# vnoz/Mutual-Information-MultiModal

Hardware: AMD Instinct MI355X
Metric: img-txt pairs/sec (MI critic fwd+bwd), global-batch InfoNCE (higher is better)
Workload: dtype bf16; 1 GPU; BASELINE configs[3]: global-batch infonce (reference semantics), bilinear critic fwd+bwd, B_global=4096, d=512; global_batch=4096, embed_dim=512, critic=bilinear, estimator=infonce, parallelism=single GPU, boundary=fp32 embeddings in, fp32 gradients out, hip_graph=False, graph_mode=none (direct C-ABI calls)

## Files before the change

mutual-information-multimodal_amd/csrc/mi_bilinear_flash.h:

```cpp
#pragma once
#include <type_traits>

#include "mi_common.h"

namespace mi {

#ifdef MI_STAMPS
#define MI_FL_STAMP(slot)                                                                       \
  do {                                                                                          \
    __builtin_amdgcn_sched_barrier(0);                                                          \
    if (threadIdx.x == 0 && g_stamps) g_stamps[(size_t)blockIdx.x * 16 + (slot)] = __builtin_amdgcn_s_memtime(); \
    __builtin_amdgcn_sched_barrier(0);                                                          \
  } while (0)
#else
#define MI_FL_STAMP(slot) do {} while (0)
#endif

#ifndef MI_FL_DIAG
#define MI_FL_DIAG 0
#endif
constexpr int kFlDiag = MI_FL_DIAG;
constexpr int kFlRows = 128;
constexpr int kFlBN = 32;
constexpr int kFlStages = 4;
constexpr float kFlThr = 60.0f;
constexpr int kFlMaxTilesPerSplit = 64;

struct FlashProblem {
  const bf16_t* q;
  const bf16_t* kv;
  const int64_t* sid_q;
  const int64_t* sid_kv;
  int64_t m, n;
  int64_t diag;
  int n_rb;
  int n_split;
  int tiles_per_split;
  const unsigned char* dup;
  float* slab;
  Partial* rec;
};
struct FlashArgs {
  FlashProblem p[2];
  int n_problems;
  int n_combo;
  int xcd_rows;
  int diag;
  int slab_f16;
  int no_index_mask;
};

template <int D>
struct FlashCfg {
  static constexpr int NK = D / 16;
  static constexpr int NT = D / 32;
  static constexpr int RB = D * 2;
  static constexpr int CPR = RB / 16;
  static constexpr int RPP = 1024 / RB;
  static constexpr int STAGE = kFlBN * RB;
  static constexpr int PIECES = STAGE / 1024 / 4;
  static constexpr int SID_OFF = kFlStages * STAGE;
  static constexpr size_t SMEM = (size_t)SID_OFF + (size_t)kFlMaxTilesPerSplit * kFlBN * 8;
  static constexpr int QA = NT >= 16 ? NK / 2 : 0;
  static constexpr int OA = NT >= 16 ? 12 : NT;
  static_assert(D == 128 || D == 256 || D == 512, "unsupported embedding width");
};

__host__ __device__ constexpr int fl_swz(int row) { return ((row & 3) << 2) | ((row >> 2) & 3); }

__device__ __forceinline__ float wave_max_uniform(float v) {
  int x;
#define MI_DPP_MAX(ctrl, rmask)                                                        \
  x = __builtin_amdgcn_update_dpp(__float_as_int(v), __float_as_int(v), ctrl, rmask, 0xF, false); \
  v = fmaxf(v, __int_as_float(x));
  MI_DPP_MAX(0xB1, 0xF)
  MI_DPP_MAX(0x4E, 0xF)
  MI_DPP_MAX(0x141, 0xF)
  MI_DPP_MAX(0x140, 0xF)
  MI_DPP_MAX(0x142, 0xA)
  MI_DPP_MAX(0x143, 0xC)
#undef MI_DPP_MAX
  return __int_as_float(__builtin_amdgcn_readlane(__float_as_int(v), 63));
}

__device__ __forceinline__ void fl_dma16(unsigned voff, const void* sbase, unsigned lds_addr) {
  unsigned keep;
  const uintptr_t b = (uintptr_t)sbase;
  const unsigned blo = __builtin_amdgcn_readfirstlane((unsigned)b), bhi = __builtin_amdgcn_readfirstlane((unsigned)(b >> 32));
  sbase = (const void*)(((uintptr_t)bhi << 32) | blo);
  lds_addr = __builtin_amdgcn_readfirstlane(lds_addr);
  asm volatile("s_mov_b32 %0, m0\n\ts_mov_b32 m0, %3\n\ts_nop 1\n\tglobal_load_lds_dwordx4 %1, %2\n\ts_mov_b32 m0, %0"
               : "=&s"(keep)
               : "v"(voff), "s"(sbase), "s"(lds_addr)
               : "memory");
}

template <int LOFF>
__device__ __forceinline__ void fl_dma_set_m0(unsigned lds_base) {
  asm volatile("s_add_u32 m0, %0, %1" : : "s"(lds_base), "n"(LOFF) : "scc");
}
template <int GOFF, int XORC>
__device__ __forceinline__ void fl_dma16_at(unsigned vlane_w, const void* sbase) {
  unsigned voff;
  asm volatile("v_xor_b32 %0, %3, %1\n\tglobal_load_lds_dwordx4 %0, %2 offset:%4"
               : "=&v"(voff)
               : "v"(vlane_w), "s"(sbase), "n"(XORC), "n"(GOFF)
               : "memory");
}

__device__ __forceinline__ float fl_max3(float a, float b, float c) {
  float d;
  asm("v_max3_f32 %0, %1, %2, %3" : "=v"(d) : "v"(a), "v"(b), "v"(c));
  return d;
}

__device__ __forceinline__ void fl_v_exp(const float& x) { asm volatile("v_exp_f32 %0, %0" : : "v"(x)); }
__device__ __forceinline__ void fl_v_add(const float& acc, const float& p) { asm volatile("v_add_f32 %0, %0, %1" : : "v"(acc), "v"(p)); }
__device__ __forceinline__ void fl_v_opaque(float& x) { asm volatile("; fl_opaque" : "+v"(x)); }
__device__ __forceinline__ unsigned fl_v_cvt_pk(const float& lo, const float& hi) {
  unsigned d;
  asm volatile("v_cvt_pk_bf16_f32 %0, %1, %2" : "=v"(d) : "v"(lo), "v"(hi));
  return d;
}
__device__ __forceinline__ void fl_v_prescale(float& x, const float& s, const float& off) {
  asm volatile("v_fmamk_f32 %0, %1, 0x3fb8aa3b, %2" : "=v"(x) : "v"(s), "v"(off));
}
__device__ __forceinline__ void fl_v_max(float& d, const float& a, const float& b) {
  asm volatile("v_max_f32 %0, %1, %2" : "=v"(d) : "v"(a), "v"(b));
}
__device__ __forceinline__ void fl_v_max3(float& d, const float& a, const float& b) {
  asm volatile("v_max3_f32 %0, %0, %1, %2" : "+v"(d) : "v"(a), "v"(b));
}
template <int STEP, bool NOP>
__device__ __forceinline__ void fl_dpp_max(const float& v) {
#define MI_FL_DPP(ctrl)                                                                            \
  if constexpr (NOP) asm volatile("s_nop 1\n\tv_max_f32_dpp %0, %0, %0 " ctrl : : "v"(v));          \
  else asm volatile("v_max_f32_dpp %0, %0, %0 " ctrl : : "v"(v))
  if constexpr (STEP == 0) { MI_FL_DPP("quad_perm:[1,0,3,2] row_mask:0xf bank_mask:0xf"); }
  else if constexpr (STEP == 1) { MI_FL_DPP("quad_perm:[2,3,0,1] row_mask:0xf bank_mask:0xf"); }
  else if constexpr (STEP == 2) { MI_FL_DPP("row_half_mirror row_mask:0xf bank_mask:0xf"); }
  else if constexpr (STEP == 3) { MI_FL_DPP("row_mirror row_mask:0xf bank_mask:0xf"); }
  else if constexpr (STEP == 4) { MI_FL_DPP("row_bcast:15 row_mask:0xa bank_mask:0xf"); }
  else { MI_FL_DPP("row_bcast:31 row_mask:0xc bank_mask:0xf"); }
#undef MI_FL_DPP
}

template <int N>
__device__ __forceinline__ void fl_wait_vmcnt_barrier() {
  asm volatile("s_waitcnt vmcnt(%0)\n\ts_barrier" ::"n"(N) : "memory");
}

template <int B, int E, class F>
__device__ __forceinline__ void fl_static_for(F&& f) {
  if constexpr (B < E) {
    f(std::integral_constant<int, B>{});
    fl_static_for<B + 1, E>(f);
  }
}

constexpr int kFlRing = 9;
constexpr int kFlAhead = 8;

template <int SLOT, int OFF>
__device__ __forceinline__ void fl_ring_read_s(bf16x8& f, int addr) {
  static_assert(OFF >= 0 && OFF < 65536, "ds offset field");
  if constexpr (SLOT == 0)
    asm volatile("ds_read_b128 v[216:219], %1 offset:%c2" : "={v[216:219]}"(f) : "v"(addr), "i"(OFF));
  else if constexpr (SLOT == 1)
    asm volatile("ds_read_b128 v[220:223], %1 offset:%c2" : "={v[220:223]}"(f) : "v"(addr), "i"(OFF));
  else if constexpr (SLOT == 2)
    asm volatile("ds_read_b128 v[224:227], %1 offset:%c2" : "={v[224:227]}"(f) : "v"(addr), "i"(OFF));
  else if constexpr (SLOT == 3)
    asm volatile("ds_read_b128 v[228:231], %1 offset:%c2" : "={v[228:231]}"(f) : "v"(addr), "i"(OFF));
  else if constexpr (SLOT == 4)
    asm volatile("ds_read_b128 v[232:235], %1 offset:%c2" : "={v[232:235]}"(f) : "v"(addr), "i"(OFF));
  else if constexpr (SLOT == 5)
    asm volatile("ds_read_b128 v[236:239], %1 offset:%c2" : "={v[236:239]}"(f) : "v"(addr), "i"(OFF));
  else if constexpr (SLOT == 6)
    asm volatile("ds_read_b128 v[240:243], %1 offset:%c2" : "={v[240:243]}"(f) : "v"(addr), "i"(OFF));
  else if constexpr (SLOT == 7)
    asm volatile("ds_read_b128 v[244:247], %1 offset:%c2" : "={v[244:247]}"(f) : "v"(addr), "i"(OFF));
  else if constexpr (SLOT == 8)
    asm volatile("ds_read_b128 v[248:251], %1 offset:%c2" : "={v[248:251]}"(f) : "v"(addr), "i"(OFF));
  else if constexpr (SLOT == 9)
    asm volatile("ds_read_b128 v[252:255], %1 offset:%c2" : "={v[252:255]}"(f) : "v"(addr), "i"(OFF));
}
template <int SLOT, int OFF_LO, int OFF_HI>
__device__ __forceinline__ void fl_ring_read_v(bf16x8& f, int addr_lo, int addr_hi) {
  static_assert(OFF_LO >= 0 && OFF_HI < 65536, "ds offset field");
  if constexpr (SLOT == 0)
    asm volatile("ds_read_b64_tr_b16 v[216:217], %1 offset:%c3\n\tds_read_b64_tr_b16 v[218:219], %2 offset:%c4"
                 : "={v[216:219]}"(f) : "v"(addr_lo), "v"(addr_hi), "i"(OFF_LO), "i"(OFF_HI));
  else if constexpr (SLOT == 1)
    asm volatile("ds_read_b64_tr_b16 v[220:221], %1 offset:%c3\n\tds_read_b64_tr_b16 v[222:223], %2 offset:%c4"
                 : "={v[220:223]}"(f) : "v"(addr_lo), "v"(addr_hi), "i"(OFF_LO), "i"(OFF_HI));
  else if constexpr (SLOT == 2)
    asm volatile("ds_read_b64_tr_b16 v[224:225], %1 offset:%c3\n\tds_read_b64_tr_b16 v[226:227], %2 offset:%c4"
                 : "={v[224:227]}"(f) : "v"(addr_lo), "v"(addr_hi), "i"(OFF_LO), "i"(OFF_HI));
  else if constexpr (SLOT == 3)
    asm volatile("ds_read_b64_tr_b16 v[228:229], %1 offset:%c3\n\tds_read_b64_tr_b16 v[230:231], %2 offset:%c4"
                 : "={v[228:231]}"(f) : "v"(addr_lo), "v"(addr_hi), "i"(OFF_LO), "i"(OFF_HI));
  else if constexpr (SLOT == 4)
    asm volatile("ds_read_b64_tr_b16 v[232:233], %1 offset:%c3\n\tds_read_b64_tr_b16 v[234:235], %2 offset:%c4"
                 : "={v[232:235]}"(f) : "v"(addr_lo), "v"(addr_hi), "i"(OFF_LO), "i"(OFF_HI));
  else if constexpr (SLOT == 5)
    asm volatile("ds_read_b64_tr_b16 v[236:237], %1 offset:%c3\n\tds_read_b64_tr_b16 v[238:239], %2 offset:%c4"
                 : "={v[236:239]}"(f) : "v"(addr_lo), "v"(addr_hi), "i"(OFF_LO), "i"(OFF_HI));
  else if constexpr (SLOT == 6)
    asm volatile("ds_read_b64_tr_b16 v[240:241], %1 offset:%c3\n\tds_read_b64_tr_b16 v[242:243], %2 offset:%c4"
                 : "={v[240:243]}"(f) : "v"(addr_lo), "v"(addr_hi), "i"(OFF_LO), "i"(OFF_HI));
  else if constexpr (SLOT == 7)
    asm volatile("ds_read_b64_tr_b16 v[244:245], %1 offset:%c3\n\tds_read_b64_tr_b16 v[246:247], %2 offset:%c4"
                 : "={v[244:247]}"(f) : "v"(addr_lo), "v"(addr_hi), "i"(OFF_LO), "i"(OFF_HI));
  else if constexpr (SLOT == 8)
    asm volatile("ds_read_b64_tr_b16 v[248:249], %1 offset:%c3\n\tds_read_b64_tr_b16 v[250:251], %2 offset:%c4"
                 : "={v[248:251]}"(f) : "v"(addr_lo), "v"(addr_hi), "i"(OFF_LO), "i"(OFF_HI));
  else if constexpr (SLOT == 9)
    asm volatile("ds_read_b64_tr_b16 v[252:253], %1 offset:%c3\n\tds_read_b64_tr_b16 v[254:255], %2 offset:%c4"
                 : "={v[252:255]}"(f) : "v"(addr_lo), "v"(addr_hi), "i"(OFF_LO), "i"(OFF_HI));
}
template <int WAIT>
__device__ __forceinline__ void fl_wait_lgkm() {
  if constexpr (kFlDiag & 16) return;
  if constexpr (WAIT >= 0) asm volatile("s_waitcnt lgkmcnt(%c0)" ::"i"(WAIT) : "memory");
}
template <bool B_IN_ACC, bool FIRST, int WAIT>
__device__ __forceinline__ void fl_mfma_s(f32x16& acc, const bf16x8& a, const bf16x8& b) {
  fl_wait_lgkm<WAIT>();
  if constexpr (FIRST) {
    if constexpr (B_IN_ACC)
      asm volatile("v_mfma_f32_32x32x16_bf16 %0, %1, %2, 0" : "=v"(acc) : "v"(a), "a"(b));
    else
      asm volatile("v_mfma_f32_32x32x16_bf16 %0, %1, %2, 0" : "=v"(acc) : "v"(a), "v"(b));
  } else {
    if constexpr (B_IN_ACC)
      asm volatile("v_mfma_f32_32x32x16_bf16 %0, %1, %2, %0" : : "v"(acc), "v"(a), "a"(b));
    else
      asm volatile("v_mfma_f32_32x32x16_bf16 %0, %1, %2, %0" : : "v"(acc), "v"(a), "v"(b));
  }
}
template <bool ACC_IN_ACC, bool NOP, int WAIT, class AT>
__device__ __forceinline__ void fl_mfma_o(f32x16& acc, const AT& a, const bf16x8& b) {
  static_assert(sizeof(AT) == 16, "a 32x32x16 bf16 operand is four registers");
  fl_wait_lgkm<WAIT>();
  if constexpr (NOP) {
    if constexpr (ACC_IN_ACC)
      asm volatile("s_nop 1\n\tv_mfma_f32_32x32x16_bf16 %0, %1, %2, %0" : "+a"(acc) : "v"(a), "v"(b));
    else
      asm volatile("s_nop 1\n\tv_mfma_f32_32x32x16_bf16 %0, %1, %2, %0" : "+v"(acc) : "v"(a), "v"(b));
  } else {
    if constexpr (ACC_IN_ACC)
      asm volatile("v_mfma_f32_32x32x16_bf16 %0, %1, %2, %0" : "+a"(acc) : "v"(a), "v"(b));
    else
      asm volatile("v_mfma_f32_32x32x16_bf16 %0, %1, %2, %0" : "+v"(acc) : "v"(a), "v"(b));
  }
}
template <bool DRAIN>
__device__ __forceinline__ void fl_score_fence(f32x16& acc) {
  if constexpr (DRAIN) asm volatile("s_nop 15\n\ts_nop 3" : "+v"(acc));
  else asm volatile("" : "+v"(acc));
}
__device__ __forceinline__ void fl_mfma_drain_all() { asm volatile("s_nop 15\n\ts_nop 3" ::: "memory"); }
template <bool IN_ACC>
__device__ __forceinline__ void fl_scale_tile(f32x16& t, float f) {
#pragma unroll
  for (int r = 0; r < 16; ++r) {
    if constexpr (IN_ACC) {
      float e = t[r], tmp;
      asm volatile("v_accvgpr_read_b32 %1, %0\n\tv_mul_f32 %1, %1, %2\n\tv_accvgpr_write_b32 %0, %1"
                   : "+a"(e), "=&v"(tmp)
                   : "v"(f));
      t[r] = e;
    } else {
      t[r] *= f;
    }
  }
}
template <bool IN_ACC>
__device__ __forceinline__ void fl_pin(bf16x8& v) {
  if constexpr (IN_ACC) asm volatile("" : "+a"(v));
  else asm volatile("" : "+v"(v));
}
template <bool IN_ACC>
__device__ __forceinline__ void fl_pin_o(f32x16& v) {
  if constexpr (IN_ACC) asm volatile("" : "+a"(v));
  else asm volatile("" : "+v"(v));
}

#ifndef MI_FL_WAIT_GROUP
#define MI_FL_WAIT_GROUP 2
#endif
constexpr int kFlWaitGroup = MI_FL_WAIT_GROUP;
template <int NS, int NV>
constexpr int fl_wait_count(int n) {
  if (n % kFlWaitGroup) return -1;
  int c = 0;
  for (int m = n + kFlWaitGroup; m <= n + kFlAhead - 1 && m < NS + NV; ++m) c += m < NS ? 1 : 2;
  return c;
}

template <int D, bool GRAD>
__global__ __launch_bounds__(256, 1) void bilinear_flash_kernel(FlashArgs args) {
  using C = FlashCfg<D>;
  extern __shared__ __attribute__((aligned(16))) char smem[];

  const FlashProblem A = args.p[0], Bp = args.p[1];
  const int n_combo = args.n_combo, n_problems = args.n_problems;
  asm volatile("" ::"s"(A.q), "s"(A.kv), "s"(A.sid_q), "s"(A.sid_kv), "s"(A.m), "s"(A.n), "s"(A.diag), "s"(A.n_rb),
               "s"(A.n_split), "s"(A.tiles_per_split), "s"(A.dup), "s"(A.slab), "s"(A.rec));
  asm volatile("" ::"s"(Bp.q), "s"(Bp.kv), "s"(Bp.sid_q), "s"(Bp.sid_kv), "s"(Bp.m), "s"(Bp.n), "s"(Bp.diag), "s"(Bp.n_rb),
               "s"(Bp.n_split), "s"(Bp.tiles_per_split), "s"(Bp.dup), "s"(Bp.slab), "s"(Bp.rec), "s"(n_combo),
               "s"(n_problems));
  const int L = (int)blockIdx.x;
  int prob, split, rb;
  if (args.xcd_rows) {
    const int ns_max = A.n_split > Bp.n_split ? A.n_split : Bp.n_split;
    const int x = L & 7, k = L >> 3;
    const int unit = x + 8 * (k / ns_max);
    split = k % ns_max;
    const int n_units = A.n_rb + (n_problems == 2 ? Bp.n_rb : 0);
    if (unit >= n_units) return;
    prob = unit >= A.n_rb ? 1 : 0;
    rb = prob ? unit - A.n_rb : unit;
    if (split >= (prob ? Bp.n_split : A.n_split)) return;
  } else {
    const int combo = L % n_combo;
    rb = L / n_combo;
    if (combo < A.n_split) {
      prob = 0;
      split = combo;
    } else if (n_problems == 2 && combo < A.n_split + Bp.n_split) {
      prob = 1;
      split = combo - A.n_split;
    } else {
      return;
    }
  }
  FlashProblem P;
  P.q = prob ? Bp.q : A.q;
  P.kv = prob ? Bp.kv : A.kv;
  P.sid_q = prob ? Bp.sid_q : A.sid_q;
  P.sid_kv = prob ? Bp.sid_kv : A.sid_kv;
  P.m = prob ? Bp.m : A.m;
  P.n = prob ? Bp.n : A.n;
  P.diag = prob ? Bp.diag : A.diag;
  P.n_rb = prob ? Bp.n_rb : A.n_rb;
  P.n_split = prob ? Bp.n_split : A.n_split;
  P.tiles_per_split = prob ? Bp.tiles_per_split : A.tiles_per_split;
  P.dup = prob ? Bp.dup : A.dup;
  P.slab = prob ? Bp.slab : A.slab;
  P.rec = prob ? Bp.rec : A.rec;
  if (rb >= P.n_rb) return;
  const int64_t n_tiles_all = P.n / kFlBN;
  const int64_t tile0 = (int64_t)split * P.tiles_per_split;
  int nt = (int)(n_tiles_all - tile0 < P.tiles_per_split ? n_tiles_all - tile0 : P.tiles_per_split);
  if (nt < 0) nt = 0;

  const int tid = threadIdx.x;
  const int wave = __builtin_amdgcn_readfirstlane(tid >> 6), lane = tid & 63;
  const int r32 = lane & 31, half = lane >> 5;
  const int64_t m_wave = (int64_t)rb * kFlRows + wave * 32;
  const bool wave_active = m_wave < P.m;
  const int64_t gi = wave_active ? m_wave + r32 : r32;
  MI_WALL_SCOPE(kWallFlash);
  MI_FL_STAMP(0);

  bf16x8 qf[C::NK];
  {
    const bf16_t* qblk = P.q + ((gi >> 5) * C::NK * 64 + lane) * 8;
#pragma unroll
    for (int kk = 0; kk < C::NK; ++kk) qf[kk] = *reinterpret_cast<const bf16x8*>(qblk + kk * 512);
  }
  const int64_t sid_i = P.sid_q[gi];
  MI_FL_STAMP(11);
  unsigned long long dupmask, diagmask;
  {
    const unsigned char* df = P.dup + (wave_active ? m_wave / 32 : 0) * n_tiles_all + tile0;
    const int flag = lane < nt ? (int)df[lane] : 0;
    dupmask = __ballot(flag == 2 || (flag == 1 && args.no_index_mask));
    diagmask = __ballot(flag == 1 && !args.no_index_mask);
  }

  const char* kv_base = reinterpret_cast<const char*>(P.kv + tile0 * kFlBN * D);
  const unsigned lds0 = (unsigned)(uintptr_t)(__attribute__((address_space(3))) char*)smem;
  const int lr = lane / C::CPR;
  const unsigned vlane = (unsigned)(lr * C::RB + 16 * ((lane % C::CPR) ^ (C::RPP > 1 ? (lr << 2) : 0)));
  auto piece_u = [](int q) __attribute__((always_inline)) {
    return C::RPP == 1 ? fl_swz(q) : (C::RPP == 2 ? (8 * (q & 1)) | ((q >> 1) & 3) : (q & 3));
  };
  const unsigned vlane_w = vlane ^ (unsigned)(16 * piece_u(C::PIECES * wave));
  auto piece_voff = [&](int i) __attribute__((always_inline)) { return vlane_w ^ (unsigned)(16 * piece_u(i)); };
  auto issue_piece = [&](int t, int i) __attribute__((always_inline)) {
    if ((kFlDiag & 1) && t >= 3) return;
    const int q = C::PIECES * wave + i;
    const int stage = t & (kFlStages - 1);
    fl_dma16(piece_voff(i), kv_base + (int64_t)t * C::STAGE + q * 1024, lds0 + stage * C::STAGE + q * 1024);
  };
  auto issue_tile = [&](int t) __attribute__((always_inline)) {
#pragma unroll
    for (int i = 0; i < C::PIECES; ++i) issue_piece(t, i);
  };
  MI_FL_STAMP(12);
  if (nt > 0) issue_tile(0);
  if (nt > 1) issue_tile(1);
  if (nt > 2) issue_tile(2);
  MI_FL_STAMP(13);

  {
    int64_t* sl = reinterpret_cast<int64_t*>(smem + C::SID_OFF);
    const int64_t* sg = P.sid_kv + tile0 * kFlBN;
    constexpr int PER = kFlMaxTilesPerSplit * kFlBN / 256;
    int64_t v[PER];
#pragma unroll
    for (int k = 0; k < PER; ++k) v[k] = tid + 256 * k < nt * kFlBN ? sg[tid + 256 * k] : 0;
#pragma unroll
    for (int k = 0; k < PER; ++k)
      if (tid + 256 * k < nt * kFlBN) sl[tid + 256 * k] = v[k];
  }

  constexpr int NO = GRAD ? C::NT : 1;
  f32x16 o[NO];
#pragma unroll
  for (int c = 0; c < NO; ++c)
#pragma unroll
    for (int r = 0; r < 16; ++r) o[c][r] = 0.0f;
  float lsum = 0.0f, pos = 0.0f;
  unsigned cnt = 0;
  float mref = MI_NEG_INF;

  const int fxh = half ^ fl_swz(r32);
  const int a0_lane = r32 * C::RB + 16 * fxh;
  const int g16 = lane >> 4, q4 = (lane & 15) >> 2, p4 = lane & 3;
  const int cl = 2 * (g16 & 1) + (p4 >> 1);
  const int a1_lane = (4 * half + q4) * C::RB + 16 * ((cl ^ half) | (q4 << 2)) + 8 * (p4 & 1);
  const int d0_wave = (int)(m_wave + P.diag - tile0 * kFlBN);

  MI_FL_STAMP(14);
  asm volatile("s_waitcnt vmcnt(0)" ::: "memory");
  MI_FL_STAMP(15);
  __syncthreads();
  MI_FL_STAMP(1);
  asm volatile("" ::"v"(sid_i), "s"(dupmask), "s"(diagmask));
  fl_static_for<0, C::NK>([&](auto KK) __attribute__((always_inline)) { fl_pin<(decltype(KK)::value < C::QA)>(qf[decltype(KK)::value]); });
  if constexpr (GRAD) fl_static_for<0, C::NT>([&](auto CT) __attribute__((always_inline)) { fl_pin_o<(decltype(CT)::value < C::OA)>(o[decltype(CT)::value]); });

  bf16x8 ring[kFlRing];
  u32x4 pfw[2];
  f32x16 s_next;
  float xs[16];
  float tA = MI_NEG_INF, tB = MI_NEG_INF, off = 0.0f;
  float f_pend = 1.0f;

  constexpr int kTailSlots = 17, kHeadSlots = 17;
  auto tail_slot = [&](auto S_) __attribute__((always_inline)) {
    constexpr int sl = decltype(S_)::value;
    if constexpr (kFlDiag & 2) return;
    if constexpr (sl < 16 && !(kFlDiag & 32)) fl_v_exp(xs[sl]);
    if constexpr (sl >= 1 && sl <= 16 && !(kFlDiag & 64)) fl_v_add(lsum, xs[sl - 1]);
    if constexpr (GRAD && sl >= 2 && sl <= 16 && sl % 2 == 0 && !(kFlDiag & 128)) {
      constexpr int k = sl / 2 - 1;
      pfw[k >> 2][k & 3] = fl_v_cvt_pk(xs[2 * k], xs[2 * k + 1]);
    }
  };
  auto decide = [&](const float& tmaxv, float thr) __attribute__((always_inline)) {
    float tmax_s, tmax_v, m_old;
    asm volatile(
        "s_nop 0\n\t"
        "v_readlane_b32 %[t], %[ta], 63\n\t"
        "v_mov_b32 %[mo], %[m]\n\t"
        "v_add_f32 %[f], %[th], %[m]\n\t"
        "v_mov_b32 %[tv], %[t]\n\t"
        "v_cmp_gt_f32 vcc, %[tv], %[f]\n\t"
        "v_sub_f32 %[f], %[m], %[tv]\n\t"
        "v_mul_f32 %[f], 0x3fb8aa3b, %[f]\n\t"
        "v_exp_f32 %[f], %[f]\n\t"
        "v_cndmask_b32 %[m], %[m], %[tv], vcc\n\t"
        "s_nop 0\n\t"
        "v_cndmask_b32 %[f], 1.0, %[f], vcc\n\t"
        "v_cmp_class_f32 vcc, %[mo], 4\n\t"
        "v_max_f32 %[o], 0xf149f2ca, %[m]\n\t"
        "v_mul_f32 %[o], 0xbfb8aa3b, %[o]\n\t"
        "v_cndmask_b32 %[f], %[f], 1.0, vcc"
        : [t] "=&s"(tmax_s), [tv] "=&v"(tmax_v), [mo] "=&v"(m_old), [f] "+v"(f_pend), [m] "+v"(mref),
          [o] "+v"(off)
        : [ta] "v"(tmaxv), [th] "s"(thr)
        : "vcc");
  };
  auto head_slot = [&](auto V_, auto NOPS_, float thr) __attribute__((always_inline)) {
    constexpr int v = decltype(V_)::value;
    constexpr bool NOPS = decltype(NOPS_)::value;
    if constexpr (kFlDiag & 2) return;
    if constexpr ((kFlDiag & 256) && v <= 10) return;
    if constexpr ((kFlDiag & 512) && v >= 11) return;
    if constexpr ((kFlDiag & 1024) && v <= 3) return;
    if constexpr ((kFlDiag & 2048) && v >= 4 && v <= 9) return;
    if constexpr ((kFlDiag & 4096) && v == 10) return;
    if constexpr (v == 0) {
      asm volatile("" : "+v"(s_next));
      cnt += 1024u;
      fl_v_max(tA, s_next[0], s_next[1]);
      fl_v_max(tB, s_next[2], s_next[3]);
    } else if constexpr (v >= 1 && v <= 3) {
      fl_v_max3(tA, s_next[4 * v], s_next[4 * v + 1]);
      fl_v_max3(tB, s_next[4 * v + 2], s_next[4 * v + 3]);
    } else if constexpr (v == 4) {
      fl_v_max(tA, tA, tB);
      fl_dpp_max<0, true>(tA);
    } else if constexpr (v >= 5 && v <= 9) {
      fl_dpp_max<v - 4, NOPS>(tA);
    } else if constexpr (v == 10) {
      decide(tA, thr);
    } else if constexpr (v >= 11 && v <= 14) {
      constexpr int r = 3 * (v - 11);
      fl_v_prescale(xs[r], s_next[r], off);
      fl_v_prescale(xs[r + 1], s_next[r + 1], off);
      fl_v_prescale(xs[r + 2], s_next[r + 2], off);
    } else if constexpr (v == 15 || v == 16) {
      constexpr int r = 12 + 2 * (v - 15);
      fl_v_prescale(xs[r], s_next[r], off);
      fl_v_prescale(xs[r + 1], s_next[r + 1], off);
    }
  };
  auto fix_masked_tile = [&](int tn) __attribute__((always_inline)) {
    unsigned mbits = 0u;
    float tq;
    unsigned long long m1;
    cnt -= 1024u;
    const int d0 = d0_wave - tn * kFlBN;
    const int want = r32 + d0 - 4 * half;
    const bool has_pos = want >= 0 && want < 32 && !(want & 4) && d0 > -32 && d0 < 32;
    const unsigned pbit = has_pos ? 1u << ((want & 3) + 4 * (want >> 3)) : 0u;
    if (__builtin_amdgcn_readfirstlane((int)((dupmask >> tn) & 1ull))) {
      MI_FL_STAMP(5);
      const int64_t* sl = reinterpret_cast<const int64_t*>(smem + C::SID_OFF) + tn * kFlBN + 4 * half;
#pragma unroll
      for (int r = 0; r < 16; ++r) {
        const bool neg = sl[(r & 3) + 8 * (r >> 2)] != sid_i;
        cnt += (unsigned)__popcll(__ballot(neg));
        mbits |= neg ? 0u : (1u << r);
        asm volatile("" : "+v"(mbits) : : "memory");
      }
      MI_FL_STAMP(6);
    } else {
      mbits = pbit;
      cnt += 1024u - 32u;
    }
    const float ninf = MI_NEG_INF;
    const float tmax_all = __int_as_float(__builtin_amdgcn_readlane(__float_as_int(tA), 63));
    const bool redo = __builtin_amdgcn_readfirstlane((int)(tmax_all > mref + kFlThr || mref == MI_NEG_INF)) != 0;
    if (!redo) {
#pragma unroll
      for (int r = 0; r < 16; r += 2) {
        unsigned t, u;
        const float s0 = s_next[r], s1 = s_next[r + 1];
        asm volatile("v_and_b32 %[t], %[b0], %[pb]\n\t"
                     "v_and_b32 %[u], %[b1], %[pb]\n\t"
                     "v_cmp_ne_u32 vcc, 0, %[t]\n\t"
                     "v_cmp_ne_u32 %[m1], 0, %[u]\n\t"
                     "v_and_b32 %[t], %[b0], %[mb]\n\t"
                     "v_and_b32 %[u], %[b1], %[mb]\n\t"
                     "v_cndmask_b32 %[q], 0, %[s0], vcc\n\t"
                     "v_add_f32 %[p], %[p], %[q]\n\t"
                     "v_cndmask_b32 %[q], 0, %[s1], %[m1]\n\t"
                     "v_add_f32 %[p], %[p], %[q]\n\t"
                     "v_cmp_ne_u32 vcc, 0, %[t]\n\t"
                     "v_cmp_ne_u32 %[m1], 0, %[u]\n\t"
                     "s_nop 1\n\t"
                     "v_cndmask_b32 %[x0], %[x0], %[ni], vcc\n\t"
                     "v_cndmask_b32 %[x1], %[x1], %[ni], %[m1]"
                     : [t] "=&v"(t), [u] "=&v"(u), [q] "=&v"(tq), [m1] "=&s"(m1), [p] "+v"(pos), [x0] "+v"(xs[r]), [x1] "+v"(xs[r + 1])
                     : [b0] "n"(1 << r), [b1] "n"(2 << r), [mb] "v"(mbits), [pb] "v"(pbit), [s0] "v"(s0), [s1] "v"(s1), [ni] "v"(ninf)
                     : "vcc");
      }
      return;
    }
    float tM = MI_NEG_INF;
#pragma unroll
    for (int r = 0; r < 16; ++r) {
      unsigned t;
      const float sr = s_next[r];
      asm volatile("v_and_b32 %[t], %[b], %[mb]\n\t"
                   "v_cmp_eq_u32 vcc, 0, %[t]\n\t"
                   "s_nop 1\n\t"
                   "v_cndmask_b32 %[t], %[ni], %[s], vcc\n\t"
                   "v_max_f32 %[tm], %[tm], %[t]\n\t"
                   "v_and_b32 %[t], %[b], %[pb]\n\t"
                   "v_cmp_ne_u32 vcc, 0, %[t]\n\t"
                   "s_nop 1\n\t"
                   "v_cndmask_b32 %[t], 0, %[s], vcc\n\t"
                   "v_add_f32 %[p], %[p], %[t]"
                   : [t] "=&v"(t), [tm] "+v"(tM), [p] "+v"(pos)
                   : [b] "n"(1 << r), [mb] "v"(mbits), [pb] "v"(pbit), [s] "v"(sr), [ni] "v"(ninf)
                   : "vcc");
    }
    float tmaxv = wave_max_uniform(tM);
    asm volatile("s_nop 1" : "+v"(tmaxv));
    decide(tmaxv, kFlThr);
#pragma unroll
    for (int r = 0; r < 16; ++r) {
      unsigned t;
      const float sr = s_next[r];
      asm volatile("v_fmamk_f32 %[x], %[s], 0x3fb8aa3b, %[o]\n\t"
                   "v_and_b32 %[t], %[b], %[mb]\n\t"
                   "v_cmp_eq_u32 vcc, 0, %[t]\n\t"
                   "s_nop 1\n\t"
                   "v_cndmask_b32 %[x], %[ni], %[x], vcc"
                   : [x] "+v"(xs[r]), [t] "=&v"(t)
                   : [b] "n"(1 << r), [mb] "v"(mbits), [s] "v"(sr), [o] "v"(off), [ni] "v"(ninf)
                   : "vcc");
    }
  };

  const unsigned long long spmask = dupmask | diagmask;

  auto iteration = [&](auto HAS_S_, auto HAS_V_, int tp) __attribute__((always_inline)) {
    constexpr bool HAS_S = decltype(HAS_S_)::value, HAS_V = decltype(HAS_V_)::value && GRAD;
    constexpr bool DO_TAIL = decltype(HAS_V_)::value;
    constexpr int NS = HAS_S ? C::NK : 0, NV = HAS_V ? 2 * C::NT : 0, NF = NS + NV;
    const bool masked_next = __builtin_amdgcn_readfirstlane((int)((spmask >> ((tp + 1) & 63)) & 1ull)) != 0;
    const float thr_next = masked_next ? __builtin_inff() : kFlThr;
    fl_v_opaque(lsum);
    if constexpr (DO_TAIL && !(kFlDiag & 2)) {
      if (__builtin_expect(__builtin_amdgcn_readfirstlane((int)__float_as_uint(f_pend)) != 0x3f800000, 0)) {
        lsum *= f_pend;
        fl_v_opaque(lsum);
        if constexpr (GRAD) {
          fl_mfma_drain_all();
          fl_static_for<0, C::NT>([&](auto CT) __attribute__((always_inline)) { fl_scale_tile<(decltype(CT)::value < C::OA)>(o[decltype(CT)::value], f_pend); });
        }
        f_pend = 1.0f;
        fl_v_opaque(f_pend);
      }
    }
    const int so = ((tp + 1) & (kFlStages - 1)) * C::STAGE + a0_lane;
    const int vo = (tp & (kFlStages - 1)) * C::STAGE + a1_lane;
    int abase[8], tbase[8];
    if constexpr (HAS_S) {
#pragma unroll
      for (int v = 0; v < 8; ++v) abase[v] = so ^ (32 * v);
    }
    if constexpr (HAS_V) {
#pragma unroll
      for (int v = 0; v < 8; ++v) tbase[v] = vo ^ (16 * ((4 * (v >> 1)) ^ (2 * (v & 1))));
    }
    auto issue_read = [&](auto NI) __attribute__((always_inline)) {
      constexpr int n = decltype(NI)::value;
      if constexpr (kFlDiag & 8) return;
      if constexpr (n < NS) {
        fl_ring_read_s<n % kFlRing, 256 * (n >> 3)>(ring[n % kFlRing], abase[n & 7]);
      } else if constexpr (n < NF) {
        constexpr int u = n - NS, ks = u / C::NT, ct = u % C::NT;
        fl_ring_read_v<n % kFlRing, 256 * (ct >> 2) + 16 * ks * C::RB, 256 * (ct >> 2) + (16 * ks + 8) * C::RB>(
            ring[n % kFlRing], tbase[2 * (ct & 3)], tbase[2 * (ct & 3) + 1]);
      }
    };
    fl_static_for<0, kFlAhead>([&](auto NI) __attribute__((always_inline)) { issue_read(NI); });
    __builtin_amdgcn_sched_barrier(0);
    fl_static_for<0, NS>([&](auto NI) __attribute__((always_inline)) {
      constexpr int n = decltype(NI)::value;
      fl_mfma_s<(n < C::QA), n == 0, fl_wait_count<NS, NV>(n)>(s_next, ring[n % kFlRing], qf[n]);
      issue_read(std::integral_constant<int, n + kFlAhead>{});
      if constexpr (DO_TAIL) {
        constexpr int NSD = NS > 0 ? NS : 1;
        constexpr int per = (kTailSlots + NSD - 1) / NSD;
        constexpr int lo = n * per, hi = (lo + per < kTailSlots ? lo + per : kTailSlots);
        fl_static_for<(lo < kTailSlots ? lo : kTailSlots), hi>([&](auto SI) __attribute__((always_inline)) { tail_slot(SI); });
      }
      __builtin_amdgcn_sched_barrier(0);
    });
    if constexpr (DO_TAIL && !HAS_S) {
      fl_static_for<0, kTailSlots>([&](auto SI) __attribute__((always_inline)) { tail_slot(SI); });
      __builtin_amdgcn_sched_barrier(0);
    }
    if constexpr (HAS_S && !HAS_V) {
      fl_score_fence<true>(s_next);
      fl_static_for<0, kHeadSlots>([&](auto VI) __attribute__((always_inline)) { head_slot(VI, std::true_type{}, thr_next); });
      __builtin_amdgcn_sched_barrier(0);
    }
    if constexpr (HAS_V) {
      constexpr int EVERY = NV / C::PIECES;
      const int tq = tp + 3 < nt ? tp + 3 : nt - 1;
      const uintptr_t gb = (uintptr_t)(kv_base + (int64_t)tq * C::STAGE + wave * (C::PIECES * 1024));
      const unsigned gb_lo = __builtin_amdgcn_readfirstlane((unsigned)gb);
      const unsigned gb_hi = __builtin_amdgcn_readfirstlane((unsigned)(gb >> 32));
      const void* sb0 = (const void*)(((uintptr_t)gb_hi << 32) | gb_lo);
      const void* sb1 = (const char*)sb0 + 4096;
      const unsigned lb = __builtin_amdgcn_readfirstlane(lds0 + (unsigned)(((tp + 3) & (kFlStages - 1)) * C::STAGE) +
                                                         (unsigned)(wave * (C::PIECES * 1024)));
      constexpr int U0 = 5;
      constexpr int n_avail = (NV - U0) - (NV / EVERY - U0 / EVERY);
      static_assert(n_avail >= 1, "no gap for the softmax head");
      fl_static_for<0, NV>([&](auto UI) __attribute__((always_inline)) {
        constexpr int u = decltype(UI)::value, n = NS + u, ks = u / C::NT, ct = u % C::NT;
        fl_mfma_o<(ct < C::OA), (u % C::NT == 0), fl_wait_count<NS, NV>(n)>(o[ct], pfw[ks], ring[n % kFlRing]);
        issue_read(std::integral_constant<int, n + kFlAhead>{});
        constexpr bool dma_gap = u % EVERY == EVERY - 1;
        if constexpr (HAS_S && u >= U0 && !dma_gap) {
          constexpr int k = (u - U0) - (u / EVERY - U0 / EVERY);
          constexpr int lo = k * kHeadSlots / n_avail, hi = (k + 1) * kHeadSlots / n_avail;
          constexpr bool nops = kHeadSlots > n_avail;
          fl_static_for<lo, hi>([&](auto VI) __attribute__((always_inline)) { head_slot(VI, std::integral_constant<bool, nops>{}, thr_next); });
        }
        if constexpr (HAS_S && !(kFlDiag & 1) && u % EVERY == EVERY - 3 && ((u / EVERY) & 3) == 0 && u / EVERY < C::PIECES)
          fl_dma_set_m0<((u / EVERY) & ~3) * 1024>(lb);
        if constexpr (dma_gap && HAS_S && !(kFlDiag & 1)) {
          constexpr int i = u / EVERY;
          fl_dma16_at<(i & 3) * 1024,
                      16 * (C::RPP == 1 ? fl_swz(i) : (C::RPP == 2 ? (8 * (i & 1)) | ((i >> 1) & 3) : (i & 3)))>(
              vlane_w, i < 4 ? sb0 : sb1);
        }
        __builtin_amdgcn_sched_barrier(0);
      });
    } else if constexpr (DO_TAIL) {
      if (tp + 3 < nt) issue_tile(tp + 3);
    }
    if constexpr (HAS_S && !(kFlDiag & 2)) {
      if (__builtin_expect(masked_next, 0)) fix_masked_tile(tp + 1);
    }
  };
  using T_ = std::true_type;
  using F_ = std::false_type;

  if (nt > 0) {
    iteration(T_{}, F_{}, -1);
    for (int t = 0; t + 1 < nt; ++t) {
      if (t == nt / 2) MI_FL_STAMP(2);
      if constexpr (kFlDiag & 4) asm volatile("s_waitcnt vmcnt(0)" ::: "memory");
      else if constexpr (GRAD) fl_wait_vmcnt_barrier<C::PIECES>();
      else if (t + 2 < nt) fl_wait_vmcnt_barrier<C::PIECES>();
      else fl_wait_vmcnt_barrier<0>();
      if (t == nt / 2) MI_FL_STAMP(3);
      iteration(T_{}, T_{}, t);
      if (t == nt / 2) MI_FL_STAMP(4);
    }
    MI_FL_STAMP(8);
    iteration(F_{}, T_{}, nt - 1);
  }
  MI_FL_STAMP(9);

  fl_v_opaque(lsum);
  lsum = wave_sum(lsum);
  pos = wave_sum(pos);
  if (lane == 0) {
    Partial rec{mref, lsum, pos, cnt};
    if (!wave_active) rec = Partial{MI_NEG_INF, 0.0f, 0.0f, 0u};
    seam_store<kSeam_FLASH>(&P.rec[((int64_t)split * P.n_rb + rb) * 4 + wave], rec);
  }
  if constexpr (GRAD) {
    fl_mfma_drain_all();
    fl_static_for<0, C::NT>([&](auto CT) __attribute__((always_inline)) { fl_pin_o<(decltype(CT)::value < C::OA)>(o[decltype(CT)::value]); });
    const int64_t wv = ((int64_t)split * P.n_rb + rb) * 4 + wave;
    if (wave_active && args.slab_f16) {
      float amax = 0.0f;
#pragma unroll
      for (int c = 0; c < C::NT; ++c)
#pragma unroll
        for (int r = 0; r < 16; ++r) amax = fmaxf(amax, __builtin_fabsf(o[c][r]));
      amax = wave_max_uniform(amax);
      int k = 13 - ((int)((__float_as_uint(amax) >> 23) & 255u) - 127);
      k = amax > 0.0f ? (k < -100 ? -100 : (k > 100 ? 100 : k)) : 0;
      const float up = __uint_as_float((unsigned)(127 + k) << 23), down = __uint_as_float((unsigned)(127 - k) << 23);
      f16_t* slab16 = reinterpret_cast<f16_t*>(P.slab);
      float* unscale = reinterpret_cast<float*>(slab16 + (int64_t)P.n_split * P.n_rb * 4 * (32 * D));
      if (lane == 0) seam_store<kSeam_FLASH>(&unscale[wv], down);
      f16_t* dst = slab16 + wv * (32 * D) + lane * 8;
#pragma unroll
      for (int c = 0; c < C::NT; ++c)
#pragma unroll
        for (int gp = 0; gp < 2; ++gp) {
          f16x8 h;
#pragma unroll
          for (int e = 0; e < 8; ++e) h[e] = (f16_t)(o[c][8 * gp + e] * up);
          seam_store<kSeam_FLASH>(reinterpret_cast<f16x8*>(dst + c * 1024 + gp * 512), h);
        }
    } else if (wave_active) {
      float* dst = P.slab + wv * (32 * D) + lane * 4;
#pragma unroll
      for (int c = 0; c < C::NT; ++c)
#pragma unroll
        for (int g = 0; g < 4; ++g) {
          const f32x4 v = {o[c][4 * g], o[c][4 * g + 1], o[c][4 * g + 2], o[c][4 * g + 3]};
          seam_store<kSeam_FLASH>(reinterpret_cast<f32x4*>(dst + c * 1024 + g * 256), v);
        }
    }
  }
  MI_FL_STAMP(10);
}

static __global__ __launch_bounds__(256) void flash_dup_flags_kernel(const int64_t* __restrict__ sid_rows,
                                                                     const int64_t* __restrict__ sid_cols, int na, int nb,
                                                                     unsigned char* __restrict__ flag,
                                                                     unsigned char* __restrict__ flag_t) {
  __shared__ int64_t rows[32];
  const int a = blockIdx.x, tid = threadIdx.x;
  if (tid < 32) rows[tid] = sid_rows[a * 32 + tid];
  __syncthreads();
  const int q = tid & 3;
  int64_t mine[8];
#pragma unroll
  for (int e = 0; e < 8; ++e) mine[e] = rows[8 * q + e];
  for (int b = blockIdx.y * 64 + (tid >> 2); b < nb; b += gridDim.y * 64) {
    const int64_t* c = sid_cols + (int64_t)b * 32;
    bool any = false;
    for (int j = 0; j < 32; ++j) {
      const int64_t v = c[j];
#pragma unroll
      for (int e = 0; e < 8; ++e) any |= v == mine[e];
    }
    int f = any ? 1 : 0;
    f |= __shfl_xor(f, 1);
    f |= __shfl_xor(f, 2);
    if (q == 0) {
      flag[(int64_t)a * nb + b] = (unsigned char)f;
      flag_t[(int64_t)b * na + a] = (unsigned char)f;
    }
  }
}

static inline int launch_flash_dup_flags(const int64_t* sid_rows, const int64_t* sid_cols, int64_t br, int64_t b,
                                         unsigned char* flag, unsigned char* flag_t, hipStream_t st) {
  const int na = (int)(br / 32), nb = (int)(b / 32);
  int gy = (nb + 63) / 64;
  if (gy > 8) gy = 8;
  {
    ProfScope prof_("bilinear equal-id tile flags", st);
    hipLaunchKernelGGL(flash_dup_flags_kernel, dim3((unsigned)na, (unsigned)gy), dim3(256), 0, st, sid_rows, sid_cols, na, nb,
                       flag, flag_t);
  }
  MI_LAUNCH_CHECK("flash_dup_flags_kernel");
  return MI_OK;
}

struct FlashReduceJob {
  const float* slab;
  const Partial* rec;
  int n_split, n_rb;
  int64_t m;
  const bf16_t* other;
  int64_t n_other, diag;
  float* out_f32;
  bf16_t* out_bf;
  bf16_t* out_bf_t;
};
struct FlashReduceArgs {
  FlashReduceJob j[2];
  const mi_stats* stats;
  const float* grad_out;
};

template <int D, bool F16>
__global__ __launch_bounds__(256) void flash_reduce_kernel(FlashReduceArgs args) {
  kernarg_prefetch<(int)sizeof(FlashReduceArgs)>();
  __shared__ float tile[32][129];
  const FlashReduceJob& J = args.j[blockIdx.z];
  const int64_t wb = blockIdx.y;
  const int cc = blockIdx.x;
  if (wb * 32 >= J.m) return;
  const int rb = (int)(wb >> 2), w = (int)(wb & 3);
  const float go = args.grad_out ? args.grad_out[0] : 1.0f;
  const float lse = args.stats->lse;
  const float gpos = go / (float)args.stats->n_pos;
  const int tid = threadIdx.x;
  float acc[16];
#pragma unroll
  for (int e = 0; e < 16; ++e) acc[e] = 0.0f;
  const int64_t i0 = wb * 32;
  const int64_t c0 = (int64_t)cc * 128;
  const int orow = tid >> 3, ocs = (tid & 7) * 16;
  const int64_t ojo = i0 + orow + J.diag;
  const bool has_other = ojo >= 0 && ojo < J.n_other;
  bf16x8 oth_a = {}, oth_b = {};
  if (has_other) {
    oth_a = *reinterpret_cast<const bf16x8*>(J.other + ojo * D + c0 + ocs);
    oth_b = *reinterpret_cast<const bf16x8*>(J.other + ojo * D + c0 + ocs + 8);
  }
  const f16_t* slab16 = reinterpret_cast<const f16_t*>(J.slab);
  const float* unscale = reinterpret_cast<const float*>(slab16 + (int64_t)J.n_split * J.n_rb * 4 * (32 * D));
  for (int s0 = 0; s0 < J.n_split; s0 += 4) {
    float cs[4];
    int64_t wvs[4];
#pragma unroll
    for (int q = 0; q < 4; ++q) {
      const int s = s0 + q < J.n_split ? s0 + q : J.n_split - 1;
      wvs[q] = ((int64_t)s * J.n_rb + rb) * 4 + w;
      const float m = J.rec[wvs[q]].m;
      cs[q] = (s0 + q < J.n_split && m > MI_NEG_INF) ? go * __expf(m - lse) * (F16 ? unscale[wvs[q]] : 1.0f) : 0.0f;
    }
    if constexpr (F16) {
      f16x8 v[4][2];
#pragma unroll
      for (int q = 0; q < 4; ++q)
#pragma unroll
        for (int u = 0; u < 2; ++u)
          v[q][u] = *reinterpret_cast<const f16x8*>(slab16 + wvs[q] * (32 * D) + (int64_t)cc * 4096 + (u * 256 + tid) * 8);
#pragma unroll
      for (int q = 0; q < 4; ++q)
        if (cs[q] != 0.0f) {
#pragma unroll
          for (int u = 0; u < 2; ++u)
#pragma unroll
            for (int e = 0; e < 8; ++e) acc[8 * u + e] += (float)v[q][u][e] * cs[q];
        }
    } else {
      f32x4 v[4][4];
#pragma unroll
      for (int q = 0; q < 4; ++q)
#pragma unroll
        for (int u = 0; u < 4; ++u)
          v[q][u] = *reinterpret_cast<const f32x4*>(J.slab + wvs[q] * (32 * D) + (int64_t)cc * 4096 + (u * 256 + tid) * 4);
#pragma unroll
      for (int q = 0; q < 4; ++q)
        if (cs[q] != 0.0f) {
#pragma unroll
          for (int u = 0; u < 4; ++u)
#pragma unroll
            for (int e = 0; e < 4; ++e) acc[4 * u + e] += v[q][u][e] * cs[q];
        }
    }
  }
  if constexpr (F16) {
#pragma unroll
    for (int u = 0; u < 2; ++u) {
      const int h = u * 256 + tid;
      const int ct_l = h >> 7, gp = (h >> 6) & 1, lane = h & 63;
      const int col = ct_l * 32 + (lane & 31);
#pragma unroll
      for (int hh = 0; hh < 2; ++hh) {
        const int row0 = 8 * (2 * gp + hh) + 4 * (lane >> 5);
#pragma unroll
        for (int e = 0; e < 4; ++e) tile[row0 + e][col] = acc[8 * u + 4 * hh + e];
      }
    }
  } else {
#pragma unroll
    for (int u = 0; u < 4; ++u) {
      const int f = u * 256 + tid;
      const int ct_l = f >> 8, g = (f >> 6) & 3, lane = f & 63;
      const int col = ct_l * 32 + (lane & 31), row0 = 8 * g + 4 * (lane >> 5);
#pragma unroll
      for (int e = 0; e < 4; ++e) tile[row0 + e][col] = acc[4 * u + e];
    }
  }
  __syncthreads();
  {
    const int row = orow, cs = ocs;
    const int64_t i = i0 + row;
    float v[16];
#pragma unroll
    for (int e = 0; e < 16; ++e) v[e] = tile[row][cs + e];
    if (has_other) {
#pragma unroll
      for (int e = 0; e < 8; ++e) {
        v[e] -= gpos * (float)oth_a[e];
        v[8 + e] -= gpos * (float)oth_b[e];
      }
#pragma unroll
      for (int e = 0; e < 16; ++e) tile[row][cs + e] = v[e];
    }
    if (J.out_f32) {
#pragma unroll
      for (int e = 0; e < 16; e += 4)
        *reinterpret_cast<f32x4*>(J.out_f32 + i * D + c0 + cs + e) = f32x4{v[e], v[e + 1], v[e + 2], v[e + 3]};
    }
    if (J.out_bf) {
      bf16x8 a, b;
#pragma unroll
      for (int e = 0; e < 8; ++e) {
        a[e] = (bf16_t)v[e];
        b[e] = (bf16_t)v[8 + e];
      }
      *reinterpret_cast<bf16x8*>(J.out_bf + i * D + c0 + cs) = a;
      *reinterpret_cast<bf16x8*>(J.out_bf + i * D + c0 + cs + 8) = b;
    }
  }
  if (J.out_bf_t) {
    __syncthreads();
    const int col = tid >> 1, rs = (tid & 1) * 16;
    bf16x8 a, b;
#pragma unroll
    for (int e = 0; e < 8; ++e) {
      a[e] = (bf16_t)tile[rs + e][col];
      b[e] = (bf16_t)tile[rs + 8 + e][col];
    }
    bf16_t* dst = J.out_bf_t + (c0 + col) * J.m + i0 + rs;
    *reinterpret_cast<bf16x8*>(dst) = a;
    *reinterpret_cast<bf16x8*>(dst + 8) = b;
  }
}

struct FlashPlan {
  bool ok;
  int n_split[2], n_rb[2], tiles_per_split[2];
  int64_t slab_bytes[2], n_rec[2];
  bool slab_f16;
};

static inline bool flash_width_ok(int64_t d) { return d == 128 || d == 256 || d == 512; }

static inline FlashPlan flash_plan(int64_t br, int64_t b, int64_t d) {
  FlashPlan fp{};
  static const bool off = getenv("MI_NO_FLASH") != nullptr;
  fp.ok = !off && flash_width_ok(d) && br % 32 == 0 && b % 32 == 0 && br >= 32;
  if (!fp.ok) return fp;
  static const bool slab_f32 = getenv("MI_FLASH_SLAB_F32") != nullptr;
  fp.slab_f16 = !slab_f32;
  const int64_t m[2] = {br, b}, n[2] = {b, br};
  int64_t total_tiles = 0;
  for (int q = 0; q < 2; ++q) {
    fp.n_rb[q] = (int)((m[q] + kFlRows - 1) / kFlRows);
    total_tiles += (int64_t)fp.n_rb[q] * (n[q] / kFlBN);
  }
  int64_t tau = (total_tiles + 255) / 256;
  if (tau < 4) tau = 4;
  if (tau > kFlMaxTilesPerSplit) tau = kFlMaxTilesPerSplit;
  if (const char* e = getenv("MI_FLASH_TILES")) tau = atoi(e) > 0 ? atoi(e) : tau;
  for (int q = 0; q < 2; ++q) {
    const int64_t tiles = n[q] / kFlBN;
    int64_t tps = tau < tiles ? tau : tiles;
    fp.n_split[q] = (int)((tiles + tps - 1) / tps);
    fp.tiles_per_split[q] = (int)((tiles + fp.n_split[q] - 1) / fp.n_split[q]);
    fp.n_split[q] = (int)((tiles + fp.tiles_per_split[q] - 1) / fp.tiles_per_split[q]);
    fp.n_rec[q] = (int64_t)fp.n_split[q] * fp.n_rb[q] * 4;
    fp.slab_bytes[q] = fp.slab_f16 ? fp.n_rec[q] * (32 * d * 2 + 4) : fp.n_rec[q] * 32 * d * 4;
  }
  return fp;
}

template <int D, bool GRAD>
static inline int launch_flash_t(const FlashArgs& a, unsigned grid, hipStream_t st, const char* what) {
  MI_SET_DYN_SMEM((bilinear_flash_kernel<D, GRAD>), FlashCfg<D>::SMEM, "hipFuncSetAttribute(bilinear_flash_kernel)");
#ifdef MI_STAMPS
  stamp_select(what, st);
#endif
  {
    ProfScope prof_(what, st);
    hipLaunchKernelGGL((bilinear_flash_kernel<D, GRAD>), dim3(grid), dim3(256), FlashCfg<D>::SMEM, st, a);
  }
  MI_LAUNCH_CHECK(what);
  return MI_OK;
}

static inline int launch_flash(FlashArgs a, int64_t d, bool grad, hipStream_t st, const char* what) {
  int combos = a.p[0].n_split + (a.n_problems == 2 ? a.p[1].n_split : 0);
  a.n_combo = (combos + 7) / 8 * 8;
  a.diag = 0;
  static const int no_index_mask = getenv("MI_FLASH_NO_INDEX_MASK") ? 1 : 0;
  a.no_index_mask = no_index_mask;
  static const int xcd_rows = getenv("MI_FLASH_XCD_COMBO") ? 0 : 1;
  a.xcd_rows = xcd_rows;
  int max_rb = a.p[0].n_rb;
  if (a.n_problems == 2 && a.p[1].n_rb > max_rb) max_rb = a.p[1].n_rb;
  unsigned grid = (unsigned)(a.n_combo * max_rb);
  if (a.xcd_rows) {
    const int ns_max = a.n_problems == 2 && a.p[1].n_split > a.p[0].n_split ? a.p[1].n_split : a.p[0].n_split;
    const int n_units = a.p[0].n_rb + (a.n_problems == 2 ? a.p[1].n_rb : 0);
    grid = (unsigned)(8 * ((n_units + 7) / 8) * ns_max);
  }
  if (d == 512) return grad ? launch_flash_t<512, true>(a, grid, st, what) : launch_flash_t<512, false>(a, grid, st, what);
  if (d == 256) return grad ? launch_flash_t<256, true>(a, grid, st, what) : launch_flash_t<256, false>(a, grid, st, what);
  if (d == 128) return grad ? launch_flash_t<128, true>(a, grid, st, what) : launch_flash_t<128, false>(a, grid, st, what);
  set_error("launch_flash: unsupported width %lld", (long long)d);
  return MI_ESHAPE;
}

static inline int launch_flash_reduce(const FlashReduceArgs& a, int n_jobs, int64_t d, bool slab_f16, hipStream_t st,
                                      const char* what) {
  int64_t mmax = a.j[0].m;
  if (n_jobs == 2 && a.j[1].m > mmax) mmax = a.j[1].m;
  dim3 grid((unsigned)(d / 128), (unsigned)(mmax / 32), (unsigned)n_jobs);
  {
    ProfScope prof_(what, st);
#define MI_FL_REDUCE(DD)                                                                                  \
  if (slab_f16) hipLaunchKernelGGL((flash_reduce_kernel<DD, true>), grid, dim3(256), 0, st, a);           \
  else hipLaunchKernelGGL((flash_reduce_kernel<DD, false>), grid, dim3(256), 0, st, a)
    if (d == 512) { MI_FL_REDUCE(512); }
    else if (d == 256) { MI_FL_REDUCE(256); }
    else { MI_FL_REDUCE(128); }
#undef MI_FL_REDUCE
  }
  MI_LAUNCH_CHECK(what);
  return MI_OK;
}

}
```

Measured before the change: 42.44 million pairs/s.

## Restructure flash kernel prologue loads and add fast path for unmasked non-redo tiles

```diff
diff --git a/mutual-information-multimodal_amd/csrc/mi_bilinear_flash.h b/mutual-information-multimodal_amd/csrc/mi_bilinear_flash.h
--- a/mutual-information-multimodal_amd/csrc/mi_bilinear_flash.h
+++ b/mutual-information-multimodal_amd/csrc/mi_bilinear_flash.h
@@ -9,7 +9,7 @@
 #define MI_FL_STAMP(slot)                                                                       \
   do {                                                                                          \
     __builtin_amdgcn_sched_barrier(0);                                                          \
-    if (threadIdx.x == 0 && g_stamps) g_stamps[(size_t)blockIdx.x * 16 + (slot)] = __builtin_amdgcn_s_memtime(); \
+    if (threadIdx.x == 0 && g_stamps) g_stamps[(size_t)blockIdx.x * 32 + (slot)] = __builtin_amdgcn_s_memtime(); \
     __builtin_amdgcn_sched_barrier(0);                                                          \
   } while (0)
 #else
@@ -306,14 +306,15 @@
 
   const FlashProblem A = args.p[0], Bp = args.p[1];
   const int n_combo = args.n_combo, n_problems = args.n_problems;
+  const int xcd_rows = args.xcd_rows, slab_f16 = args.slab_f16, no_index_mask = args.no_index_mask;
   asm volatile("" ::"s"(A.q), "s"(A.kv), "s"(A.sid_q), "s"(A.sid_kv), "s"(A.m), "s"(A.n), "s"(A.diag), "s"(A.n_rb),
                "s"(A.n_split), "s"(A.tiles_per_split), "s"(A.dup), "s"(A.slab), "s"(A.rec));
   asm volatile("" ::"s"(Bp.q), "s"(Bp.kv), "s"(Bp.sid_q), "s"(Bp.sid_kv), "s"(Bp.m), "s"(Bp.n), "s"(Bp.diag), "s"(Bp.n_rb),
                "s"(Bp.n_split), "s"(Bp.tiles_per_split), "s"(Bp.dup), "s"(Bp.slab), "s"(Bp.rec), "s"(n_combo),
-               "s"(n_problems));
+               "s"(n_problems), "s"(xcd_rows), "s"(slab_f16), "s"(no_index_mask));
   const int L = (int)blockIdx.x;
   int prob, split, rb;
-  if (args.xcd_rows) {
+  if (xcd_rows) {
     const int ns_max = A.n_split > Bp.n_split ? A.n_split : Bp.n_split;
     const int x = L & 7, k = L >> 3;
     const int unit = x + 8 * (k / ns_max);
@@ -365,21 +366,32 @@
   MI_WALL_SCOPE(kWallFlash);
   MI_FL_STAMP(0);
 
+  const int64_t sid_i = P.sid_q[gi];
+  int flag_raw;
+  {
+    const unsigned char* df = P.dup + (wave_active ? m_wave / 32 : 0) * n_tiles_all;
+    int64_t ft = tile0 + (lane < nt ? lane : (nt > 0 ? nt - 1 : 0));
+    ft = ft < n_tiles_all ? ft : n_tiles_all - 1;
+    asm volatile("global_load_ubyte %0, %1, off" : "=&v"(flag_raw) : "v"(df + ft) : "memory");
+  }
+  constexpr int PER = kFlMaxTilesPerSplit * kFlBN / 256;
+  int64_t sidv[PER];
+  {
+    int64_t id_last = tile0 * kFlBN + (nt > 0 ? nt * kFlBN - 1 : 0);
+    id_last = id_last < P.n ? id_last : P.n - 1;
+#pragma unroll
+    for (int k = 0; k < PER; ++k) {
+      const int64_t j = tile0 * kFlBN + tid + 256 * k;
+      sidv[k] = P.sid_kv[j < id_last ? j : id_last];
+    }
+  }
   bf16x8 qf[C::NK];
   {
     const bf16_t* qblk = P.q + ((gi >> 5) * C::NK * 64 + lane) * 8;
 #pragma unroll
     for (int kk = 0; kk < C::NK; ++kk) qf[kk] = *reinterpret_cast<const bf16x8*>(qblk + kk * 512);
   }
-  const int64_t sid_i = P.sid_q[gi];
   MI_FL_STAMP(11);
-  unsigned long long dupmask, diagmask;
-  {
-    const unsigned char* df = P.dup + (wave_active ? m_wave / 32 : 0) * n_tiles_all + tile0;
-    const int flag = lane < nt ? (int)df[lane] : 0;
-    dupmask = __ballot(flag == 2 || (flag == 1 && args.no_index_mask));
-    diagmask = __ballot(flag == 1 && !args.no_index_mask);
-  }
 
   const char* kv_base = reinterpret_cast<const char*>(P.kv + tile0 * kFlBN * D);
   const unsigned lds0 = (unsigned)(uintptr_t)(__attribute__((address_space(3))) char*)smem;
@@ -390,33 +402,19 @@
   };
   const unsigned vlane_w = vlane ^ (unsigned)(16 * piece_u(C::PIECES * wave));
   auto piece_voff = [&](int i) __attribute__((always_inline)) { return vlane_w ^ (unsigned)(16 * piece_u(i)); };
-  auto issue_piece = [&](int t, int i) __attribute__((always_inline)) {
+  auto issue_piece = [&](int t, int src, int i) __attribute__((always_inline)) {
     if ((kFlDiag & 1) && t >= 3) return;
     const int q = C::PIECES * wave + i;
     const int stage = t & (kFlStages - 1);
-    fl_dma16(piece_voff(i), kv_base + (int64_t)t * C::STAGE + q * 1024, lds0 + stage * C::STAGE + q * 1024);
+    fl_dma16(piece_voff(i), kv_base + (int64_t)src * C::STAGE + q * 1024, lds0 + stage * C::STAGE + q * 1024);
   };
-  auto issue_tile = [&](int t) __attribute__((always_inline)) {
-#pragma unroll
-    for (int i = 0; i < C::PIECES; ++i) issue_piece(t, i);
+  auto issue_tile = [&](int t, int src) __attribute__((always_inline)) {
+#pragma unroll
+    for (int i = 0; i < C::PIECES; ++i) issue_piece(t, src, i);
   };
   MI_FL_STAMP(12);
-  if (nt > 0) issue_tile(0);
-  if (nt > 1) issue_tile(1);
-  if (nt > 2) issue_tile(2);
+  if (nt > 0) issue_tile(0, 0);
   MI_FL_STAMP(13);
-
-  {
-    int64_t* sl = reinterpret_cast<int64_t*>(smem + C::SID_OFF);
-    const int64_t* sg = P.sid_kv + tile0 * kFlBN;
-    constexpr int PER = kFlMaxTilesPerSplit * kFlBN / 256;
-    int64_t v[PER];
-#pragma unroll
-    for (int k = 0; k < PER; ++k) v[k] = tid + 256 * k < nt * kFlBN ? sg[tid + 256 * k] : 0;
-#pragma unroll
-    for (int k = 0; k < PER; ++k)
-      if (tid + 256 * k < nt * kFlBN) sl[tid + 256 * k] = v[k];
-  }
 
   constexpr int NO = GRAD ? C::NT : 1;
   f32x16 o[NO];
@@ -424,6 +422,7 @@
   for (int c = 0; c < NO; ++c)
 #pragma unroll
     for (int r = 0; r < 16; ++r) o[c][r] = 0.0f;
+  if constexpr (GRAD) fl_static_for<0, C::NT>([&](auto CT) __attribute__((always_inline)) { fl_pin_o<(decltype(CT)::value < C::OA)>(o[decltype(CT)::value]); });
   float lsum = 0.0f, pos = 0.0f;
   unsigned cnt = 0;
   float mref = MI_NEG_INF;
@@ -436,13 +435,28 @@
   const int d0_wave = (int)(m_wave + P.diag - tile0 * kFlBN);
 
   MI_FL_STAMP(14);
-  asm volatile("s_waitcnt vmcnt(0)" ::: "memory");
+  asm volatile("s_waitcnt vmcnt(0)" : "+v"(flag_raw) : : "memory");
   MI_FL_STAMP(15);
+  unsigned long long dupmask, diagmask;
+  {
+    const int flag = lane < nt ? flag_raw : 0;
+    dupmask = __ballot(flag == 2 || (flag == 1 && no_index_mask));
+    diagmask = __ballot(flag == 1 && !no_index_mask);
+  }
+  {
+    int64_t* sl = reinterpret_cast<int64_t*>(smem + C::SID_OFF);
+#pragma unroll
+    for (int k = 0; k < PER; ++k) sl[tid + 256 * k] = sidv[k];
+  }
   __syncthreads();
   MI_FL_STAMP(1);
   asm volatile("" ::"v"(sid_i), "s"(dupmask), "s"(diagmask));
   fl_static_for<0, C::NK>([&](auto KK) __attribute__((always_inline)) { fl_pin<(decltype(KK)::value < C::QA)>(qf[decltype(KK)::value]); });
-  if constexpr (GRAD) fl_static_for<0, C::NT>([&](auto CT) __attribute__((always_inline)) { fl_pin_o<(decltype(CT)::value < C::OA)>(o[decltype(CT)::value]); });
+  if (nt > 1) {
+    issue_tile(1, 1);
+    issue_tile(2, nt > 2 ? 2 : 1);
+  }
+  MI_FL_STAMP(18);
 
   bf16x8 ring[kFlRing];
   u32x4 pfw[2];
@@ -530,7 +544,8 @@
     const int want = r32 + d0 - 4 * half;
     const bool has_pos = want >= 0 && want < 32 && !(want & 4) && d0 > -32 && d0 < 32;
     const unsigned pbit = has_pos ? 1u << ((want & 3) + 4 * (want >> 3)) : 0u;
-    if (__builtin_amdgcn_readfirstlane((int)((dupmask >> tn) & 1ull))) {
+    const bool general = __builtin_amdgcn_readfirstlane((int)((dupmask >> tn) & 1ull)) != 0;
+    if (general) {
       MI_FL_STAMP(5);
       const int64_t* sl = reinterpret_cast<const int64_t*>(smem + C::SID_OFF) + tn * kFlBN + 4 * half;
 #pragma unroll
@@ -548,6 +563,26 @@
     const float ninf = MI_NEG_INF;
     const float tmax_all = __int_as_float(__builtin_amdgcn_readlane(__float_as_int(tA), 63));
     const bool redo = __builtin_amdgcn_readfirstlane((int)(tmax_all > mref + kFlThr || mref == MI_NEG_INF)) != 0;
+    if (!redo && !general) {
+      const unsigned eidx = has_pos ? (unsigned)((want & 3) + 4 * (want >> 3)) : ~0u;
+#pragma unroll
+      for (int r = 0; r < 16; r += 2) {
+        const float s0 = s_next[r], s1 = s_next[r + 1];
+        asm volatile("v_cmp_eq_u32 vcc, %[r0], %[e]\n\t"
+                     "v_cmp_eq_u32 %[m1], %[r1], %[e]\n\t"
+                     "s_nop 0\n\t"
+                     "v_cndmask_b32 %[q], 0, %[s0], vcc\n\t"
+                     "v_cndmask_b32 %[x0], %[x0], %[ni], vcc\n\t"
+                     "v_add_f32 %[p], %[p], %[q]\n\t"
+                     "v_cndmask_b32 %[q], 0, %[s1], %[m1]\n\t"
+                     "v_cndmask_b32 %[x1], %[x1], %[ni], %[m1]\n\t"
+                     "v_add_f32 %[p], %[p], %[q]"
+                     : [q] "=&v"(tq), [m1] "=&s"(m1), [p] "+v"(pos), [x0] "+v"(xs[r]), [x1] "+v"(xs[r + 1])
+                     : [r0] "n"(r), [r1] "n"(r + 1), [e] "v"(eidx), [s0] "v"(s0), [s1] "v"(s1), [ni] "v"(ninf)
+                     : "vcc");
+      }
+      return;
+    }
     if (!redo) {
 #pragma unroll
       for (int r = 0; r < 16; r += 2) {
@@ -712,7 +747,7 @@
         __builtin_amdgcn_sched_barrier(0);
       });
     } else if constexpr (DO_TAIL) {
-      if (tp + 3 < nt) issue_tile(tp + 3);
+      if (tp + 3 < nt) issue_tile(tp + 3, tp + 3);
     }
     if constexpr (HAS_S && !(kFlDiag & 2)) {
       if (__builtin_expect(masked_next, 0)) fix_masked_tile(tp + 1);
@@ -746,17 +781,19 @@
     if (!wave_active) rec = Partial{MI_NEG_INF, 0.0f, 0.0f, 0u};
     seam_store<kSeam_FLASH>(&P.rec[((int64_t)split * P.n_rb + rb) * 4 + wave], rec);
   }
+  MI_FL_STAMP(16);
   if constexpr (GRAD) {
     fl_mfma_drain_all();
     fl_static_for<0, C::NT>([&](auto CT) __attribute__((always_inline)) { fl_pin_o<(decltype(CT)::value < C::OA)>(o[decltype(CT)::value]); });
     const int64_t wv = ((int64_t)split * P.n_rb + rb) * 4 + wave;
-    if (wave_active && args.slab_f16) {
+    if (wave_active && slab_f16) {
       float amax = 0.0f;
 #pragma unroll
       for (int c = 0; c < C::NT; ++c)
 #pragma unroll
         for (int r = 0; r < 16; ++r) amax = fmaxf(amax, __builtin_fabsf(o[c][r]));
       amax = wave_max_uniform(amax);
+      MI_FL_STAMP(17);
       int k = 13 - ((int)((__float_as_uint(amax) >> 23) & 255u) - 127);
       k = amax > 0.0f ? (k < -100 ? -100 : (k > 100 ? 100 : k)) : 0;
       const float up = __uint_as_float((unsigned)(127 + k) << 23), down = __uint_as_float((unsigned)(127 - k) << 23);
```

After: 42.73 million pairs/s (median of 6 runs). No clear change (+0.7%).
